# cvlab-kaist/SOLA

Hardware: AMD Instinct MI355X
Metric: track-selection forward+loss samples/sec at (T=32,N=64,d=256) (higher is better)
Workload: dtype f32 via split-f16 (hi+lo f16 operand pairs, 3 f16 MFMAs per product, f32 accumulate); 1 GPU; SOLA track selection forward+BCE+alignment loss+selection, T=32 N=64 d=256 L=16, mevis/default model (32.98M params, random init), 256 samples/step/GPU, conv weights re-standardised every step; batch_per_gpu=256, tracks=64, frames=32, text_len=16

## Files before the change

### include/sola_hip.h

```cpp
#ifndef SOLA_HIP_H
#define SOLA_HIP_H

#include <stddef.h>
#include <stdint.h>

#ifdef __cplusplus
extern "C" {
#endif

typedef enum SolaStatus {
    SOLA_OK = 0,
    SOLA_ERR_ARG = -1,
    SOLA_ERR_HIP = -2,
    SOLA_ERR_WEIGHT = -3,
    SOLA_ERR_WORKSPACE = -4,
    SOLA_ERR_STATE = -5
} SolaStatus;

typedef struct SolaConfig {
    int32_t object_token_dim;
    int32_t lang_token_dim;
    int32_t n_layers;
    int32_t max_temporal_length;
    int32_t n_negative;
    int32_t n_groups;
    int32_t n_groups_module;
    int32_t num_heads;
} SolaConfig;

typedef struct SolaCtx SolaCtx;

const char* sola_last_error(void);
const char* sola_version(void);

int sola_ctx_create(const SolaConfig* cfg, int device, SolaCtx** out);
int sola_ctx_destroy(SolaCtx* ctx);

int sola_num_weights(const SolaCtx* ctx);
int sola_weight_info(const SolaCtx* ctx, int index, const char** name, int64_t* numel);

int sola_set_weight(SolaCtx* ctx, const char* name, const void* dev_ptr, int64_t numel);

int sola_weights_changed(SolaCtx* ctx);
int sola_set_ws_policy(SolaCtx* ctx, int recompute_every_forward);

int sola_set_precision(SolaCtx* ctx, int precision);
int sola_set_split_guard(SolaCtx* ctx, int enable);

int sola_set_x16_arena(SolaCtx* ctx, void* dev_ptr, size_t bytes);
int sola_x16_arena_info(const SolaCtx* ctx, size_t* need_bytes, size_t* capacity_bytes, size_t* used_bytes);
int sola_split_fallback_count(const SolaCtx* ctx, int64_t* count, int32_t* last_guard);
int sola_cast_sp16(const float* dev_in, int ld_in, float* dev_out, int ld_out, int64_t rows, int K, float scale, void* stream);
int sola_cast_sp16_auto(const float* dev_in, int ld_in, float* dev_out, int ld_out, int64_t rows, int K, float* dev_scal, void* stream);
int sola_gemm_nt_split(const float* dev_a_sp, int lda, const float* dev_w_sp, const float* dev_bias, const float* dev_r,
                       int ldr, int r_is_split, float* dev_c, int ldc, int c_is_split, int M, int N, int K, float out_scale,
                       void* stream);
int sola_gemm_nt_split_scaled(const float* dev_a_sp, int lda, const float* dev_w_sp, const float* dev_bias, const float* dev_r,
                              int ldr, int r_is_split, float* dev_c, int ldc, int c_is_split, int M, int N, int K,
                              float out_scale, const float* dev_out_scale, void* stream);

int sola_cast_f16(const float* dev_in, int ld_in, void* dev_out, int ld_out, int64_t rows, int K, float scale, float* dev_scal, void* stream);
int sola_gemm_nt_f16(const void* dev_a_h, int lda, const void* dev_w_h, const float* dev_bias, const void* dev_r_h, int ldr,
                     void* dev_c, int ldc, int c_is_f16, int M, int N, int K, float out_scale, void* stream);
int sola_attention_f16(const void* dev_q, int ldq, const void* dev_k, int ldk, const void* dev_v, int ldv, void* dev_o, int ldo,
                       int G, int H, int head_dim, int Sq, int Sk, int inner, int64_t q_outer, int64_t q_inner, int64_t q_row_stride,
                       int64_t k_outer, int64_t k_inner, int64_t k_row_stride, float scale, void* stream);

int sola_gemm_nt_bf16(const void* dev_a, int lda, const void* dev_w, const float* dev_bias, const void* dev_r, int ldr, int r_is_bf16,
                      void* dev_c, int ldc, int c_is_bf16, int M, int N, int K, void* stream);
int sola_attention_bf16(const void* dev_q, int ldq, const void* dev_k, int ldk, const void* dev_v, int ldv, float* dev_o, void* dev_o_bf16, int ldo,
// ... 228 lines not shown
```

### sola_amd/_lib.py

```python
from __future__ import annotations

import contextlib
import ctypes as C
import os

_HERE = os.path.dirname(os.path.abspath(__file__))
LIB_PATH = os.environ.get("SOLA_HIP_LIB") or os.path.join(_HERE, "lib", "libsola_hip.so")


class SolaLibraryError(RuntimeError):
    pass


class SolaError(RuntimeError):
    """A libsola_hip call returned a negative status."""


class SolaConfig(C.Structure):
    _fields_ = [
        ("object_token_dim", C.c_int32),
        ("lang_token_dim", C.c_int32),
        ("n_layers", C.c_int32),
        ("max_temporal_length", C.c_int32),
        ("n_negative", C.c_int32),
# ... 8 lines not shown
        ("n_videos", C.c_int32),
        ("video_tracks", C.POINTER(C.c_int32)),
        ("video_frames", C.POINTER(C.c_int32)),
        ("n_samples", C.c_int32),
        ("sample_video", C.POINTER(C.c_int32)),
        ("sample_text_len", C.POINTER(C.c_int32)),
    ]


_vp, _i, _i64, _f, _sz = C.c_void_p, C.c_int, C.c_int64, C.c_float, C.c_size_t

SIGNATURES = {
    "sola_last_error": (C.c_char_p, []),
    "sola_version": (C.c_char_p, []),
    "sola_ctx_create": (_i, [C.POINTER(SolaConfig), _i, C.POINTER(_vp)]),
    "sola_ctx_destroy": (_i, [_vp]),
    "sola_num_weights": (_i, [_vp]),
    "sola_weight_info": (_i, [_vp, _i, C.POINTER(C.c_char_p), C.POINTER(_i64)]),
    "sola_set_weight": (_i, [_vp, C.c_char_p, _vp, _i64]),
    "sola_weights_changed": (_i, [_vp]),
    "sola_set_ws_policy": (_i, [_vp, _i]),
    "sola_set_precision": (_i, [_vp, _i]),
    "sola_set_split_guard": (_i, [_vp, _i]),
    "sola_split_fallback_count": (_i, [_vp, C.POINTER(_i64), C.POINTER(C.c_int32)]),
    "sola_cast_sp16": (_i, [_vp, _i, _vp, _i, _i64, _i, _f, _vp]),
    "sola_gemm_nt_split": (_i, [_vp, _i, _vp, _vp, _vp, _i, _i, _vp, _i, _i, _i, _i, _i, _f, _vp]),
    "sola_cast_sp16_auto": (_i, [_vp, _i, _vp, _i, _i64, _i, _vp, _vp]),
    "sola_gemm_nt_split_scaled": (_i, [_vp, _i, _vp, _vp, _vp, _i, _i, _vp, _i, _i, _i, _i, _i, _f, _vp, _vp]),
    "sola_cast_f16": (_i, [_vp, _i, _vp, _i, _i64, _i, _f, _vp, _vp]),
    "sola_gemm_nt_f16": (_i, [_vp, _i, _vp, _vp, _vp, _i, _vp, _i, _i, _i, _i, _i, _f, _vp]),
    "sola_gemm_nn": (_i, [_vp, _i, _vp, _vp, _vp, _i, _vp, _i, _vp, _i, _i, _i, _i, _vp]),
    "sola_gemm_nt_bf16": (_i, [_vp, _i, _vp, _vp, _vp, _i, _i, _vp, _i, _i, _i, _i, _i, _vp]),
    "sola_attention_bf16": (_i, [_vp, _i, _vp, _i, _vp, _i, _vp, _vp, _i, _i, _i, _i, _i, _i, _i, _i64, _i64, _i64, _i64, _i64, _i64, _f, _vp, _vp]),
    "sola_attention_backward_bf16": (_i, [_vp, _i, _vp, _i, _vp, _i, _vp, _i, _vp, _i, _i, _vp, _vp, _vp, _vp, _i, _i, _i, _vp, _vp, _i, _i, _i, _i, _i, _i,
                                          _i64, _i64, _i64, _i64, _i64, _i64, _f, _i64, _vp, _sz, _vp]),
    "sola_attention_f16": (_i, [_vp, _i, _vp, _i, _vp, _i, _vp, _i, _i, _i, _i, _i, _i, _i, _i64, _i64, _i64, _i64, _i64, _i64, _f, _vp]),
    "sola_workspace_bytes": (_sz, [_vp, _i, _i, _i, _i]),
    "sola_forward": (_i, [_vp, _vp, _vp, _i, _i, _i, _i, _vp, _vp, _vp, _sz, _vp]),
    "sola_ragged_workspace_bytes": (_sz, [_vp, C.POINTER(SolaRaggedBatch)]),
    "sola_forward_ragged": (_i, [_vp, _vp, _vp, C.POINTER(SolaRaggedBatch), _vp, _vp, _vp, _sz, _vp]),
    "sola_loss_ragged": (_i, [_vp, _vp, _vp, _vp, _vp, _i64, _i, _vp, _i, _i64, _i, _i, _f, _f, _f, _vp, _vp, _vp, _sz, _vp]),
    "sola_train_ragged_workspace_bytes": (_sz, [_vp, C.POINTER(SolaRaggedBatch)]),
    "sola_backward_ragged_workspace_bytes": (_sz, [_vp, C.POINTER(SolaRaggedBatch)]),
    "sola_forward_train_ragged": (_i, [_vp, _vp, _vp, C.POINTER(SolaRaggedBatch), _vp, _vp, _vp, _sz, _vp]),
    "sola_backward_ragged": (_i, [_vp, _vp, _vp, _vp, _vp, _sz, _vp]),
    "sola_loss_backward_ragged": (_i, [_vp, _vp, _vp, _vp, _vp, _i64, _i, _vp, _i, _i64, _i, _i, _f, _f, _f, _vp, _vp, _vp, _vp, _vp, _sz, _vp]),
# ... 179 lines not shown
```

### sola_amd/csrc/api.hip

```cpp
#include <math.h>
#include <stdarg.h>
#include <string.h>

#include <algorithm>
#include <exception>
#include <mutex>

#include "ragged.h"
#include "tune.h"

static thread_local char g_err[1024] = "";
void sola_set_error(const char* fmt, ...) {
    va_list ap;
    va_start(ap, fmt);
    vsnprintf(g_err, sizeof(g_err), fmt, ap);
    va_end(ap);
}
extern "C" const char* sola_last_error(void) { return g_err; }
extern "C" const char* sola_version(void) { return "sola_hip 0.6 (gfx950; f32, range-guarded split-f16 and f16-operand MFMA forward and backward, ragged batches, mask IoU + masklet rows)"; }

namespace {
struct ProfRec {
    int cat;
    hipEvent_t e0, e1;
// ... 577 lines not shown
                                const float* neg, int64_t neg_batch_stride, int n_samples, const int32_t* dev_track_offsets,
                                int max_tracks, int64_t total_tracks, int D, int n_neg, float pw, float temperature, float aw,
                                float* loss3, int32_t* neg_argmax, void* scratch, size_t scratch_bytes, void* stream_) {
    SOLA_ARG(score_map && score_tokens && labels && pos && neg && loss3 && scratch && dev_track_offsets, "loss_ragged: null argument");
    SOLA_ARG(n_samples > 0 && max_tracks > 0 && total_tracks > 0 && D > 0 && n_neg > 0, "loss_ragged: bad sizes");
    const size_t need = (size_t)total_tracks * 3 * sizeof(float);
    if (scratch_bytes < need) {
        sola_set_error("loss_ragged: scratch %zu bytes < required %zu", scratch_bytes, need);
        return SOLA_ERR_WORKSPACE;
    }
    LossDesc d{};
    d.score_map = score_map; d.score_tokens = score_tokens; d.labels = labels; d.pos = pos;
    d.neg = neg; d.neg_batch_stride = neg_batch_stride;
    d.B = n_samples; d.N = max_tracks; d.D = D; d.n_neg = n_neg;
    d.pos_w = pw; d.temp_scale = expf(temperature); d.align_w = aw;
    d.terms = static_cast<float*>(scratch); d.loss3 = loss3; d.neg_argmax = neg_argmax;
    d.trk_off = dev_track_offsets;
    return launch_loss(d, as_stream(stream_));
}

extern "C" int sola_set_split_guard(SolaCtx* c, int enable) {
    SOLA_ARG(c, "set_split_guard: null ctx");
    c->split_guard = enable != 0;
    return SOLA_OK;
}

extern "C" int sola_set_x16_arena(SolaCtx* c, void* dev_ptr, size_t bytes) {
    SOLA_ARG(c, "set_x16_arena: null ctx");
    SOLA_ARG((reinterpret_cast<uintptr_t>(dev_ptr) & 255) == 0, "set_x16_arena: the arena must be 256-byte aligned");
    c->x16.clear();
    c->x16_arena = static_cast<char*>(dev_ptr);
    c->x16_cap = dev_ptr ? bytes : 0;
    c->x16_used = 0;
    if (!dev_ptr) c->x16_need = 0;
    return SOLA_OK;
}

extern "C" int sola_x16_arena_info(const SolaCtx* c, size_t* need_bytes, size_t* capacity_bytes, size_t* used_bytes) {
    SOLA_ARG(c, "x16_arena_info: null ctx");
    if (need_bytes) *need_bytes = c->x16_need;
    if (capacity_bytes) *capacity_bytes = c->x16_cap;
    if (used_bytes) *used_bytes = c->x16_used;
    return SOLA_OK;
}

extern "C" int sola_split_fallback_count(const SolaCtx* c, int64_t* count, int32_t* last_guard) {
// ... 556 lines not shown
```

### sola_amd/csrc/backward.hip

```cpp
#include <math.h>
#include <stdlib.h>

#include <algorithm>
#include <initializer_list>
#include <string>
#include <vector>

#include "ragged.h"

extern int g_train_split_min_rows;
int g_bwd_dual_cast = 1;
int g_bwd_fused_bf16_cast = 1;

int g_train_dw_f16 = 1;
int g_bwd_side_rows = 0;
int g_bwd_group_rows = 2048;

namespace {

struct Arena {
    char* base;
    size_t total = 0;
    std::unordered_map<std::string, size_t> off, bytes;
    size_t add(const std::string& name, size_t floats) {
// ... 164 lines not shown
    const int max_rows_smp = rt ? rt->maxRowsSample : N * Tp;
    const float scale = 1.0f / sqrtf((float)DH);
    float* tn = ar.get("tn");
    const size_t tn_bytes = ar.total - ar.off.at("tn");
    float* wt = ar.get("wt");
    float* const splitk_ws = ar.off.count("splitk") ? ar.get("splitk") : nullptr;
    const size_t splitk_bytes = splitk_ws ? (size_t)8192 * 4096 * sizeof(float) : 0;
    const bool split = c->precision >= 1 && ar.off.count("dy_sp") != 0;
    const bool pure = c->precision >= 2;
    const int bf = c->precision == 3 ? 1 : 0;
    const int lowp_arith = pure ? 2 : 1;
    const bool dw16 = !pure && g_train_dw_f16 != 0;
    auto cast_scaled = [&](const float* in, int ld, float* out, long long rows, int K, float* scal) -> int {
        return pure ? launch_cast_f16_scaled(in, ld, out, K, rows, K, scal, s, bf) : launch_cast_sp16_scaled(in, ld, out, K, rows, K, scal, s);
    };
    auto cast_auto = [&](const float* in, int ld, float* out, long long rows, int K, float* scal) -> int {
        return pure ? launch_cast_f16(in, ld, out, K, rows, K, 0.f, scal, s, 13, nullptr, bf) : launch_cast_sp16_auto(in, ld, out, K, rows, K, scal, s);
    };
    auto cast_fixed = [&](const float* in, int ld, float* out, long long rows, int K, float scale) -> int {
        return pure ? launch_cast_f16(in, ld, out, K, rows, K, scale, nullptr, s, 13, nullptr, bf) : launch_cast_sp16(in, ld, out, K, rows, K, scale, s);
    };

    const bool lane_on = !split && g_bwd_side_rows > 0 && M <= g_bwd_side_rows;
    if (lane_on && !c->side_stream) {
        SOLA_HIP(hipStreamCreateWithFlags(&c->side_stream, hipStreamNonBlocking));
        SOLA_HIP(hipEventCreateWithFlags(&c->ev_fork, hipEventDisableTiming));
        for (hipEvent_t& e : c->ev_side) SOLA_HIP(hipEventCreateWithFlags(&e, hipEventDisableTiming));
    }
    hipStream_t s2 = lane_on ? c->side_stream : s;
    const bool group = !split && !lane_on && ar.off.count("dwkeep") != 0;
    float* keep_ptr = group ? ar.get("dwkeep") : nullptr;
    auto keep = [&](size_t floats) { float* q = keep_ptr; keep_ptr += (floats + 63) & ~(size_t)63; return q; };
    GemmTnGroupDesc gq{};
    auto flush_group = [&]() -> int {
        if (gq.nprob == 0) return SOLA_OK;
        SOLA_TRY(launch_gemm_tn_group(gq, s));
        gq.nprob = 0;
        return SOLA_OK;
    };
    const float* nn_w[3] = {nullptr, nullptr, nullptr};
    int nn_rows = 0;
    bool side_pending[4] = {false, false, false, false};
    auto dw_begin = [&]() -> int {
        if (!lane_on) return SOLA_OK;
        SOLA_HIP(hipEventRecord(c->ev_fork, s));
        SOLA_HIP(hipStreamWaitEvent(s2, c->ev_fork, 0));
        return SOLA_OK;
    };
    auto dw_end = [&](int slot) -> int {
        if (!lane_on) return SOLA_OK;
        SOLA_HIP(hipEventRecord(c->ev_side[slot], s2));
// ... 621 lines not shown
```

### sola_amd/csrc/ctx.h

```cpp
#pragma once
#include <string>
#include <unordered_map>
#include <vector>

#include "kernels.h"

struct ConvGeom {
    int cin, cout, k, stride, pad;
};
struct Weight {
    std::string name;
    int64_t numel;
    const float* ptr;
    float* grad;
};
struct Buf {
    size_t off;
    int64_t rows, cols;
};
struct Plan {
    int B = 0, N = 0, T = 0, L = 0, W = 0, Tp = 0, M = 0;
    int Tl[6] = {0};
    bool train = false;
    bool rag = false;
// ... 58 lines not shown
    void* x16_alloc(size_t bytes) {
        bytes = (bytes + 255) & ~(size_t)255;
        x16_need += bytes;
        if (x16_used + bytes > x16_cap) return nullptr;
        void* r = x16_arena + x16_used;
        x16_used += bytes;
        return r;
    }
    const void* x16_find(const float* src, int cols, int fmt) const {
        for (const X16Entry& e : x16)
            if (e.src == src && e.cols == cols && e.fmt == fmt) return e.p16;
        return nullptr;
    }
    float* scal_buf = nullptr;
    int* guard = nullptr;
    int* guard_host = nullptr;
    bool split_guard = true;
    long long split_fallbacks = 0;
    bool weight_range_bad = false;
    SolaRagStage* rag_stage = nullptr;
    std::vector<hipEvent_t> bucket_ev;
    hipStream_t side_stream = nullptr;
    hipEvent_t ev_fork = nullptr, ev_side[4] = {nullptr, nullptr, nullptr, nullptr};
    bool bucket_recorded = false;
    int n_buckets() const { return cfg.n_layers + 1; }
    float* scal_pair(int i) const { return scal_buf + 2 * i; }
    float* scal_extra(int i) const { return scal_buf + 2 * (2 + (size_t)cfg.n_layers * 12) + 2 + i; }
    const float* lin_inv_scale(int layer, int attn, int proj) const { return scal_buf + 2 * (2 + (layer * 3 + attn) * 4 + proj) + 1; }
    struct StepBinding {
        std::vector<int> widx;
        std::vector<int32_t> group;
        std::vector<long long> numel;
        int n_groups = 0;
        size_t sq_scratch = 0;
    } step;
    void* adam_tab = nullptr;
    int adam_n = 0, adam_cap = 0, adam_blocks = 0;
    bool adam_has_steps = false;
    int* adam_ticket = nullptr;
    double adam_bytes = 0.0;
    float p_drop_encoder = 0.f, p_drop_attention = 0.f;
    unsigned long long drop_seed = 0;
    DropoutCfg enc_drop(int conv_idx) const { return make_dropout(p_drop_encoder, drop_seed, 1u + (unsigned)conv_idx); }
    DropoutCfg attn_drop(int layer, int a) const { return make_dropout(p_drop_attention, drop_seed, 100u + 3u * (unsigned)layer + (unsigned)a); }
};

static const int kConvIdx[6] = {0, 4, 8, 12, 16, 20};
static const int kNormIdx[5] = {1, 5, 9, 13, 17};
static const char* const kAttnShort[3] = {"obj", "mot", "o2l"};
static const char* const kAttnLong[3] = {"obj_attn", "motion_attn", "object2lang_attn"};
constexpr float kLinScale = 64.f;
int sola_refresh_lin16(SolaCtx* c, hipStream_t s);
int sola_refresh_conv_weights(SolaCtx* c, int fmt, bool force, hipStream_t s);
int sola_check_forward_args(const SolaCtx* c, const char* who, size_t need, const void* workspace, size_t ws_bytes);

inline const float* ctx_weight(const SolaCtx* c, const std::string& name) {
    auto it = c->index.find(name);
    return it == c->index.end() ? nullptr : c->weights[it->second].ptr;
}
inline float* ctx_grad(const SolaCtx* c, const std::string& name) {
    auto it = c->index.find(name);
    return it == c->index.end() ? nullptr : c->weights[it->second].grad;
}

inline std::string abuf(bool train, int layer, const char* attn, const char* what) {
    if (!train) return what;
    return "l" + std::to_string(layer) + "_" + attn + "_" + what;
}

struct RagShape;
Plan make_plan(const SolaCtx* c, int B, int N, int T, int L, bool train);
Plan make_plan_ragged(const SolaCtx* c, const RagShape& r, bool train);
int sola_forward_train_impl(SolaCtx* c, const float* obj, const float* lang, int B, int N, int T, int L, float* score_map,
                            float* score_tokens, void* workspace, size_t ws_bytes, hipStream_t s, const RagShape* rs = nullptr);
int sola_forward_infer_impl(SolaCtx* c, const float* obj, const float* lang, int B, int N, int T, int L, float* score_map,
                            float* score_tokens, void* workspace, size_t ws_bytes, hipStream_t s);
// ... 5 lines not shown
```

### sola_amd/csrc/forward.hip

```cpp
#include <math.h>
#include <string.h>

#include <algorithm>

#include "ragged.h"

int g_train_gn_cast = 1;
extern int g_train_dw_f16;
int g_train_attn_cast = 1;
int g_train_bf16_store = 3;
int g_train_gn_stats = 1;
int g_train_x16_keep = 1;
int g_train_split_min_rows = 1024;

namespace {
struct PlanSizes {
    int64_t rows0;
    int64_t rows[6];
    int64_t M, BW;
    int64_t S;
    int64_t gn_slots;
    size_t tables;
};
void plan_fill(Plan& p, const SolaCtx* c, const PlanSizes& z, bool train) {
// ... 43 lines not shown
        p.add("l" + std::to_string(l) + "_o2l", z.M, D);
    }
}
}

Plan make_plan(const SolaCtx* c, int B, int N, int T, int L, bool train) {
    Plan p;
    p.B = B; p.N = N; p.T = T; p.L = L; p.train = train;
    p.W = L + c->cfg.n_negative;
    int t = T;
    for (int i = 0; i < 6; ++i) {
        t = (t + 2 * c->conv[i].pad - c->conv[i].k) / c->conv[i].stride + 1;
        p.Tl[i] = t;
    }
    p.Tp = p.Tl[5];
    p.M = B * N * p.Tp;
    const int64_t R = (int64_t)B * N;
    PlanSizes z{};
    z.rows0 = R * T;
    for (int i = 0; i < 6; ++i) z.rows[i] = R * p.Tl[i];
    z.M = p.M; z.BW = (int64_t)B * p.W; z.S = B;
    z.gn_slots = std::max<int64_t>(R * T, (int64_t)p.M) / 4 + 1024;
    plan_fill(p, c, z, train);
    return p;
}

Plan make_plan_ragged(const SolaCtx* c, const RagShape& r, bool train) {
    Plan p;
    p.rag = true;
    p.B = r.S; p.N = r.maxN; p.T = r.maxT[0]; p.L = r.maxW - c->cfg.n_negative; p.train = train;
    p.W = r.maxW;
    for (int i = 0; i < 6; ++i) p.Tl[i] = r.maxT[i + 1];
    p.Tp = r.maxT[6];
    p.M = (int)r.Ms;
    PlanSizes z{};
    z.rows0 = r.rows[0];
    for (int i = 0; i < 6; ++i) z.rows[i] = r.rows[i + 1];
    z.M = r.Ms; z.BW = r.LW; z.S = r.S;
    z.gn_slots = (int64_t)(rag_gn_slots_bytes(r) / 4 + 64);
    z.tables = rag_tables_bytes(r, train);
    plan_fill(p, c, z, train);
    return p;
}

int sola_forward_train_impl(SolaCtx* c, const float* obj, const float* lang, int B, int N, int T, int L, float* score_map,
                            float* score_tokens, void* workspace, size_t ws_bytes, hipStream_t s, const RagShape* rs) {
// ... 351 lines not shown
```

### sola_amd/csrc/forward_infer.hip

```cpp
#include <math.h>

#include <algorithm>

#include "ctx.h"

int sola_refresh_lin16(SolaCtx* c, hipStream_t s) {
    if (!c->lin16_dirty) return SOLA_OK;
    SOLA_ARG(c->lin16_buf && c->scal_buf, "split-f16 weights requested before sola_set_precision(ctx, 1)");
    static const char* pn[4] = {"q_proj", "k_proj", "v_proj", "out_proj"};
    const int D = c->cfg.lang_token_dim;
    std::vector<const float*> in;
    std::vector<float*> out;
    for (int l = 0; l < c->cfg.n_layers; ++l)
        for (int a = 0; a < 3; ++a)
            for (int j = 0; j < 4; ++j) {
                const std::string nm = "object_lang_align_layers." + std::to_string(l) + "." + kAttnLong[a] + "." + pn[j] + ".weight";
                const float* w = ctx_weight(c, nm);
                if (!w) {
                    sola_set_error("forward: weight '%s' has not been set", nm.c_str());
                    return SOLA_ERR_WEIGHT;
                }
                in.push_back(w);
                out.push_back(c->lin16_buf + ((size_t)(l * 3 + a) * 4 + j) * D * D);
            }
// ... 46 lines not shown
    c->ws16_fmt = fmt;
    return SOLA_OK;
}

int sola_check_forward_args(const SolaCtx* c, const char* who, size_t need, const void* workspace, size_t ws_bytes) {
    for (const Weight& w : c->weights)
        if (!w.ptr) {
            sola_set_error("%s: weight '%s' has not been set", who, w.name.c_str());
            return SOLA_ERR_WEIGHT;
        }
    if (ws_bytes < need) {
        sola_set_error("%s: workspace %zu bytes < required %zu", who, ws_bytes, need);
        return SOLA_ERR_WORKSPACE;
    }
    SOLA_ARG((reinterpret_cast<uintptr_t>(workspace) & 255) == 0, "%s: workspace must be 256-byte aligned", who);
    return SOLA_OK;
}

int g_attn_split_min_keys = 96;

int g_lang_shared_neg = 1;

int launch_attention_f16(const AttnDesc& d, hipStream_t s);

int sola_forward_infer_impl(SolaCtx* c, const float* obj, const float* lang, int B, int N, int T, int L, float* score_map,
                            float* score_tokens, void* workspace, size_t ws_bytes, hipStream_t s) {
    SOLA_ARG(c && obj && lang && score_map && score_tokens && workspace, "forward: null argument");
    SOLA_ARG(B > 0 && N > 0 && T > 0 && L >= 1, "forward: bad sizes B=%d N=%d T=%d L=%d", B, N, T, L);
    const bool sp = c->precision == 1;
    const bool h16 = c->precision == 2;
    if (sp)
        SOLA_ARG(c->cfg.object_token_dim % 8 == 0 && (c->cfg.lang_token_dim / c->cfg.n_groups_module) % 8 == 0 &&
                     (2 * c->cfg.object_token_dim / c->cfg.n_groups) % 8 == 0 && (c->cfg.lang_token_dim / c->cfg.n_groups) % 8 == 0,
                 "split-f16 mode needs channel counts per GroupNorm group that are multiples of 8");
    if (h16)
        SOLA_ARG(c->cfg.object_token_dim % 64 == 0 && c->cfg.lang_token_dim % 64 == 0,
                 "16-bit storage mode needs object_token_dim and lang_token_dim to be multiples of 64");
    Plan p = make_plan(c, B, N, T, L, false);
    SOLA_TRY(sola_check_forward_args(c, "forward", p.total, workspace, ws_bytes));
    char* base = static_cast<char*>(workspace);
    auto buf = [&](const std::string& name) { return reinterpret_cast<float*>(base + p.bufs.at(name).off); };
    float* const splitk_ws = (!h16 && p.bufs.count("splitk")) ? buf("splitk") : nullptr;
    const size_t splitk_bytes = splitk_ws ? (size_t)p.bufs.at("splitk").rows * p.bufs.at("splitk").cols * sizeof(float) : 0;
    auto W = [&](const std::string& name) { return ctx_weight(c, name); };
    const int D = c->cfg.lang_token_dim, H = c->cfg.num_heads, DH = D / H, d_in = c->cfg.object_token_dim;
    const int Tp = p.Tp, M = p.M, Wn = p.W;
    const int R = B * N;
    int* const guard = (sp || h16) ? c->guard : nullptr;
    auto ws_w = [&](int i) -> const float* {
        if (h16) return reinterpret_cast<const float*>(reinterpret_cast<const _Float16*>(c->ws16_buf) + c->ws_off[i]);
        return sp ? c->ws16_buf + c->ws_off[i] : c->ws_buf + c->ws_off[i];
    };
    auto lin_w = [&](const std::string& an, const char* proj_name, int layer, int attn, int proj) -> const float* {
        const size_t idx = (size_t)(layer * 3 + attn) * 4 + proj;
        if (sp) return c->lin16_buf + idx * D * D;
        if (h16) return reinterpret_cast<const float*>(reinterpret_cast<const _Float16*>(c->lin16_buf) + idx * D * D);
        return W(an + "." + proj_name + ".weight");
    };
    auto lin_inv = [&](int layer, int attn, int proj) -> const float* { return (sp || h16) ? c->lin_inv_scale(layer, attn, proj) : nullptr; };

    SOLA_TRY(sola_refresh_conv_weights(c, sp ? 1 : (h16 ? 2 : 0), false, s));
    if (sp || h16) {
        SOLA_TRY(sola_refresh_lin16(c, s));
        SOLA_HIP(hipMemsetAsync(c->guard, 0, sizeof(int), s));
    } else {
        c->x16.clear();
        c->x16_used = 0;
        c->x16_need = 0;
    }

    const float* x = obj;
    if (sp) SOLA_TRY(launch_cast_sp16_auto(obj, d_in, buf("obj_sp"), d_in, (long long)R * T, d_in, c->scal_pair(0), s));
    if (h16) SOLA_TRY(launch_cast_f16(obj, d_in, buf("obj_sp"), d_in, (long long)R * T, d_in, 256.f, c->scal_pair(0), s, 6, c->scal_extra(0)));
    if (sp || h16) x = buf("obj_sp");
    const bool conv5_16 = h16 || (sp && c->conv[5].cout % 8 == 0);
    int t_in = T;
    for (int i = 0; i < 6; ++i) {
        const ConvGeom& g = c->conv[i];
        const std::string cp = "short_motion_encoder." + std::to_string(kConvIdx[i]);
        const bool to16 = i == 5 && conv5_16;
        GemmDesc gd{};
        gd.nprob = 1;
        gd.p[0] = GemmProblem{x, ws_w(i), W(cp + ".bias"), nullptr, to16 ? buf("conv5_sp") : buf("conv" + std::to_string(i))};
        gd.M = R * p.Tl[i]; gd.N = g.cout; gd.K = g.k * g.cin;
        gd.lda = g.cin; gd.ldr = 0; gd.ldc = g.cout;
        gd.conv = g.k > 1 ? 1 : 0;
        gd.T_in = t_in; gd.T_out = p.Tl[i]; gd.stride = g.stride; gd.pad = g.pad; gd.Cin = g.cin;
        if (sp) {
            gd.arith = 1; gd.out_scale = 1.f; gd.c_sp16 = to16 ? 1 : 0; gd.guard = guard;
            if (i == 0) gd.out_scale_dev = c->scal_pair(0) + 1;
        }
        if (h16) {
            gd.arith = 2; gd.out_scale = 1.f; gd.c_f16 = 1; gd.guard = guard;
            if (i == 0) gd.bias_scale_dev = c->scal_extra(0);
        }
        gd.splitk_ws = splitk_ws; gd.splitk_bytes = splitk_bytes;
        bool fused_norm = false;
// ... 10 lines not shown
            }
        }
        SOLA_TRY(launch_gemm(gd, s));
        if (i < 5 && !fused_norm) {
            const std::string np = "short_motion_encoder." + std::to_string(kNormIdx[i]);
            GroupNormDesc nd{};
            nd.slice_ws = buf("gn_slots"); nd.slice_ws_bytes = (size_t)p.bufs.at("gn_slots").rows * p.bufs.at("gn_slots").cols * sizeof(float);
            nd.x = buf("conv" + std::to_string(i)); nd.y = buf("act" + std::to_string(i));
            nd.gamma = W(np + ".weight"); nd.beta = W(np + ".bias");
            nd.n_inst = R; nd.inner = 1; nd.outer_stride = p.Tl[i]; nd.inner_stride = 0; nd.tok_stride = 1;
            nd.ntok = p.Tl[i]; nd.C = g.cout; nd.groups = c->cfg.n_groups; nd.eps = 1e-5f; nd.slope = 0.01f; nd.leaky = 1;
            nd.out_sp16 = sp ? 1 : 0; nd.guard = guard;
            if (h16) {
                nd.in_f16 = 1; nd.out_f16 = 1;
                if (i == 0) nd.in_scale_dev = c->scal_pair(0) + 1;
            }
            SOLA_TRY(launch_group_norm(nd, s));
        }
        if (i < 5) x = buf("act" + std::to_string(i));
        t_in = p.Tl[i];
    }
    if (sp && !conv5_16) SOLA_TRY(launch_cast_sp16(buf("conv5"), D, buf("conv5_sp"), D, M, D, 1.f, s));

    SOLA_TRY(launch_pos_encoding(W("positional_encoding_gaussian_matrix"), D, Tp, c->cfg.max_temporal_length, buf("pe"), s));
    bool shared_neg = false;
    if (sp && g_lang_shared_neg && c->cfg.n_negative > 0 && Wn <= g_attn_split_min_keys && (long long)B * L + c->cfg.n_negative >= 1024) {
        AttnDesc probe{};
        probe.G = B; probe.H = H; probe.DH = DH; probe.Sq = N * Tp; probe.Sk = Wn; probe.inner = 1; probe.k_private = L;
        shared_neg = attention_shared_keys_supported(probe);
    }
    const long long lang_rows = shared_neg ? (long long)B * L + c->cfg.n_negative : (long long)B * Wn;
    if (shared_neg) SOLA_TRY(launch_lang_concat_shared(lang, W("negative_token.weight"), buf("lang"), buf("lbar"), B, L, c->cfg.n_negative, D, s));
    else SOLA_TRY(launch_lang_concat(lang, W("negative_token.weight"), buf("lang"), buf("lbar"), B, L, c->cfg.n_negative, D, s));
    if (sp) SOLA_TRY(launch_cast_sp16_auto(buf("lang"), D, buf("lang_sp"), D, lang_rows, D, c->scal_pair(1), s));
    if (h16) SOLA_TRY(launch_cast_f16(buf("lang"), D, buf("lang_sp"), D, lang_rows, D, 1.f, c->scal_pair(1), s, 6));
    const float* const lang_in = (sp || h16) ? buf("lang_sp") : buf("lang");

    const float scale = 1.0f / sqrtf((float)DH);
    auto linear3 = [&](const float* a0, const float* a1, const float* a2, int layer, int attn, int nprob, int rows, float* o0,
                       float* o1, float* o2, int first_proj, int out_sp16, const float* a_inv_scale = nullptr) -> int {
        static const char* pn[3] = {"q_proj", "k_proj", "v_proj"};
        const std::string an = "object_lang_align_layers." + std::to_string(layer) + "." + kAttnLong[attn];
        const float* as[3] = {a0, a1, a2};
        float* os[3] = {o0, o1, o2};
        GemmDesc gd{};
        gd.nprob = nprob;
        for (int j = 0; j < nprob; ++j)
            gd.p[j] = GemmProblem{as[j], lin_w(an, pn[first_proj + j], layer, attn, first_proj + j), W(an + "." + pn[first_proj + j] + ".bias"),
                                  nullptr, os[j], lin_inv(layer, attn, first_proj + j)};
        gd.M = rows; gd.N = D; gd.K = D; gd.lda = D; gd.ldr = 0; gd.ldc = D;
        if (sp) { gd.arith = 1; gd.out_scale = 1.f; gd.out_scale_dev = a_inv_scale; gd.c_sp16 = out_sp16; gd.guard = guard; }
        if (h16) { gd.arith = 2; gd.out_scale = 1.f; gd.out_scale_dev = a_inv_scale; gd.c_f16 = 1; gd.guard = guard; }
        gd.splitk_ws = splitk_ws; gd.splitk_bytes = splitk_bytes;
        return launch_gemm(gd, s);
    };
    auto out_proj = [&](int layer, int attn, const float* resid, int resid_sp16) -> int {
        const std::string an = "object_lang_align_layers." + std::to_string(layer) + "." + kAttnLong[attn];
        GemmDesc gd{};
        gd.nprob = 1;
        gd.p[0] = GemmProblem{buf("attn"), lin_w(an, "out_proj", layer, attn, 3), W(an + ".out_proj.bias"), resid, buf("res"), lin_inv(layer, attn, 3)};
        gd.M = M; gd.N = D; gd.K = D; gd.lda = D; gd.ldr = D; gd.ldc = D;
        if (sp) { gd.arith = 1; gd.out_scale = 1.f; gd.r_sp16 = resid_sp16; }
        if (h16) { gd.arith = 2; gd.out_scale = 1.f; gd.r_f16 = 1; gd.c_f16 = 1; gd.guard = guard; }
        gd.splitk_ws = splitk_ws; gd.splitk_bytes = splitk_bytes;
        return launch_gemm(gd, s);
    };
    auto gn = [&](const std::string& lp, int idx, float* y, float* y2, int out16, int n_inst, int inner, long long outer,
                  long long inner_stride, long long tok_stride, int ntok) -> int {
        GroupNormDesc nd{};
        nd.slice_ws = buf("gn_slots"); nd.slice_ws_bytes = (size_t)p.bufs.at("gn_slots").rows * p.bufs.at("gn_slots").cols * sizeof(float);
        nd.x = buf("res"); nd.y = y; nd.y2 = y2; nd.pe = y2 ? buf("pe") : nullptr;
        nd.gamma = W(lp + "norm." + std::to_string(idx) + ".weight");
        nd.beta = W(lp + "norm." + std::to_string(idx) + ".bias");
        nd.n_inst = n_inst; nd.inner = inner; nd.outer_stride = outer; nd.inner_stride = inner_stride;
        nd.tok_stride = tok_stride; nd.ntok = ntok; nd.C = D; nd.groups = c->cfg.n_groups_module;
        nd.eps = 1e-5f; nd.slope = 0.f; nd.leaky = 0; nd.guard = guard;
        if (sp) nd.out_sp16 = out16;
        if (h16) { nd.in_f16 = 1; nd.out_f16 = out16; }
        return launch_group_norm(nd, s);
    };
    auto attention = [&](const float* q, const float* k, const float* v, int G, int Sq, int Sk, int inner, long long qo,
                         long long qi, long long qr, long long ko, long long ki, long long kr, int in_sp16, int k_private = 0,
                         long long k_shared_row = 0) -> int {
        AttnDesc ad{q, k, v, buf("attn"), D, D, D, D, G, H, DH, Sq, Sk, inner, qo, qi, qr, ko, ki, kr, scale, nullptr};
        ad.k_private = k_private;
        ad.k_shared_row = k_shared_row;
        ad.o_sp16 = sp ? 1 : 0;
        ad.in_sp16 = in_sp16;
        ad.guard = guard;
        ad.split_math = sp ? 1 : 0;
        return h16 ? launch_attention_f16(ad, s) : launch_attention(ad, s);
    };
    const int obj_sp = (sp && N > g_attn_split_min_keys && N > 16 && DH % 16 == 0) ? 1 : 0;
    const int mot_sp = (sp && Tp > g_attn_split_min_keys && Tp > 16 && DH % 16 == 0) ? 1 : 0;
    const int o2l_sp = (sp && Wn > g_attn_split_min_keys && DH % 16 == 0) ? 1 : 0;

    const float* xin = (sp || h16) ? buf("conv5_sp") : buf("conv5");
    const float* xres = conv5_16 ? buf("conv5_sp") : buf("conv5");
    int xres_sp = conv5_16 ? 1 : 0;
    for (int l = 0; l < c->cfg.n_layers; ++l) {
        const std::string lp = "object_lang_align_layers." + std::to_string(l) + ".";
        const std::string ls = "l" + std::to_string(l);
        const bool last = l + 1 == c->cfg.n_layers;
        float *q = buf("q"), *k = buf("k"), *v = buf("v");
        float* x_obj = buf(ls + "_obj");
        float* x_pe = buf(ls + "_xpe");
        float* x_mot = buf(ls + "_motion");
        float* x_o2l = buf(ls + "_o2l");
        SOLA_TRY(linear3(xin, xin, xin, l, 0, 3, M, q, k, v, 0, obj_sp));
        SOLA_TRY(attention(q, k, v, B * Tp, N, N, Tp, (long long)N * Tp, 1, Tp, (long long)N * Tp, 1, Tp, obj_sp));
        SOLA_TRY(out_proj(l, 0, xres, xres_sp));
        SOLA_TRY(gn(lp, 0, x_obj, x_pe, 1, B * Tp, Tp, (long long)N * Tp, 1, Tp, N));
        SOLA_TRY(linear3(x_pe, x_pe, x_obj, l, 1, 3, M, q, k, v, 0, mot_sp));
        SOLA_TRY(attention(q, k, v, B * N, Tp, Tp, 1, (long long)Tp, 0, 1, (long long)Tp, 0, 1, mot_sp));
        SOLA_TRY(out_proj(l, 1, x_obj, 1));
        SOLA_TRY(gn(lp, 1, x_mot, nullptr, 1, B * N, 1, Tp, 0, 1, Tp));
        SOLA_TRY(linear3(x_mot, nullptr, nullptr, l, 2, 1, M, q, nullptr, nullptr, 0, o2l_sp));
        SOLA_TRY(linear3(lang_in, lang_in, nullptr, l, 2, 2, (int)lang_rows, buf("lk"), buf("lv"), nullptr, 1, o2l_sp, c->scal_pair(1) + 1));
        if (shared_neg) SOLA_TRY(attention(q, buf("lk"), buf("lv"), B, N * Tp, Wn, 1, (long long)N * Tp, 0, 1, (long long)L, 0, 1, o2l_sp, L, (long long)B * L));
        else SOLA_TRY(attention(q, buf("lk"), buf("lv"), B, N * Tp, Wn, 1, (long long)N * Tp, 0, 1, (long long)Wn, 0, 1, o2l_sp));
        SOLA_TRY(out_proj(l, 2, x_mot, 1));
        SOLA_TRY(gn(lp, 2, x_o2l, nullptr, last ? 0 : 1, B, 1, (long long)N * Tp, 0, 1, N * Tp));
        xin = x_o2l;
        xres = x_o2l;
        xres_sp = 1;
    }

    HeadDesc hd{xin, buf("lbar"), score_map, score_tokens, B, N, Tp, D};
    SOLA_TRY(launch_score_head(hd, s));
    c->last = p;
    c->last_obj = nullptr;
    return SOLA_OK;
}
```

### sola_amd/module.py

```python
from __future__ import annotations

import ctypes as C

import os

import torch
import torch.nn as nn

from . import _lib
from ._lib import SolaConfig, SolaError, SolaRaggedBatch, check, current_stream, lib, ptr, require_cuda

NUM_HEADS = 8


class _AttentionParams(nn.Module):

    def __init__(self, embed_dim, num_heads, dropout_p=0.1):
        super().__init__()
        self.embed_dim, self.num_heads, self.dropout_p = embed_dim, num_heads, dropout_p
        self.q_proj = nn.Linear(embed_dim, embed_dim)
        self.k_proj = nn.Linear(embed_dim, embed_dim)
        self.v_proj = nn.Linear(embed_dim, embed_dim)
        self.out_proj = nn.Linear(embed_dim, embed_dim)

# ... 62 lines not shown
        mods = []
        for cin, cout, k, s, pad in geo:
            mods += [nn.Conv1d(cin, cout, kernel_size=k, stride=s, padding=pad),
                     nn.GroupNorm(self.n_groups, cout), nn.LeakyReLU(), nn.Dropout(p=p)]
        mods.append(nn.Conv1d(D, D, kernel_size=1, stride=1, padding=0))
        self.short_motion_encoder = nn.Sequential(*mods)
        self.object_lang_align_layers = nn.ModuleList([ObjectLanguageAlignmentLayer(configs) for _ in range(self.n_layers)])
        self.register_buffer("positional_encoding_gaussian_matrix", torch.randn((1, D // 2)).float())
        self.negative_token = nn.Embedding(self.n_negative, D)
        self._ctx = None
        self._ctx_device = None
        self._bound = {}
        self._weights_touched = False
        self._workspace = None
        self._last_shape = None
        self.ws_policy = "auto"
        self.attention_dropout_p = 0.1
        env = os.environ.get("SOLA_PRECISION")
        self._precision = env or "f16x3"
        self.train_precision = os.environ.get("SOLA_TRAIN_PRECISION") or env or "f32"
        self._ctx_precision = None
        self.split_guard = True
        self._ctx_guard = None
        self._train_ws = None
        self._bwd_ws = None
        self._train_inputs = None
        self._train_shape = None
        self._train_generation = 0
        self._grad_arena = None
        self._grad_ctx = None
        self._grad_bound = None
        self._grads_in_arena = False

    def _config_struct(self):
        return SolaConfig(self.object_token_dim, self.lang_token_dim, self.n_layers, self.max_temporal_length,
                          self.n_negative, self.n_groups, self.n_groups_module, NUM_HEADS)

    def _ensure_ctx(self, device):
        if self._ctx is not None and self._ctx_device == device:
            return
        self._release_ctx()
        handle = C.c_void_p()
        cfg = self._config_struct()
        check(lib().sola_ctx_create(C.byref(cfg), device.index if device.index is not None else torch.cuda.current_device(),
                                    C.byref(handle)), "sola_ctx_create")
        self._ctx, self._ctx_device, self._bound = handle, device, {}
        self._ctx_precision = None
        self._ctx_guard = None

    def _release_ctx(self):
        if getattr(self, "_ctx", None) is not None:
            try:
                lib().sola_ctx_destroy(self._ctx)
            finally:
                self._ctx = None

    def __del__(self):
        try:
            self._release_ctx()
        except Exception:
            pass

    def _params(self):
        return [(key, owner._parameters[leaf]) for key, owner, leaf, is_buf in self._state_entries() if not is_buf]

    def _param_list(self):
        return [p for _, p in self._params()]

    def _state_entries(self):
        se = self.__dict__.get("_state_cache")
        if se is None:
# ... 29 lines not shown
            rec = (t.data_ptr(), t._version)
            old = self._bound.get(key)
            if old is None or old[0] != rec[0]:
                check(lib().sola_set_weight(self._ctx, key.encode(), ptr(t), t.numel()), f"sola_set_weight({key})")
                self._adam_sig = None
                changed = True
            elif old[1] != rec[1]:
                changed = True
            self._bound[key] = rec
        if changed:
            check(lib().sola_weights_changed(self._ctx), "sola_weights_changed")
        every = self.training if self.ws_policy == "auto" else self.ws_policy == "always"
        check(lib().sola_set_ws_policy(self._ctx, 1 if every else 0), "sola_set_ws_policy")
        prec = self.train_precision if train else self._precision
        if prec not in ("f32", "f16x3", "f16", "bf16"):
            raise SolaError(f"precision must be 'f32', 'f16x3', 'f16' or 'bf16', got {prec!r}")
        want = {"f32": 0, "f16x3": 1, "f16": 2, "bf16": 3 if train else 1}[prec]
        if self._ctx_precision != want:
            check(lib().sola_set_precision(self._ctx, want), "sola_set_precision")
            self._ctx_precision = want
        if self._ctx_guard != bool(self.split_guard):
            check(lib().sola_set_split_guard(self._ctx, 1 if self.split_guard else 0), "sola_set_split_guard")
            self._ctx_guard = bool(self.split_guard)

    def split_fallbacks(self):
        if self._ctx is None:
            return 0, 0
        n, g = C.c_int64(), C.c_int32()
        check(lib().sola_split_fallback_count(self._ctx, C.byref(n), C.byref(g)), "sola_split_fallback_count")
        return int(n.value), int(g.value)

    def _get_workspace(self, nbytes, device):
        if self._workspace is None or self._workspace.numel() < nbytes or self._workspace.device != device:
            self._workspace = torch.empty(int(nbytes), dtype=torch.uint8, device=device)
        return self._workspace

    def _check_inputs(self, object_tokens, lang_tokens):
        if object_tokens.dim() != 4 or lang_tokens.dim() != 3:
            raise SolaError("object_tokens must be [B,N,T,d] and lang_tokens [B,L,D]")
        B, N, T, d = object_tokens.shape
        Bl, L, D = lang_tokens.shape
        if d != self.object_token_dim or D != self.lang_token_dim or Bl != B:
            raise SolaError(f"shape mismatch: object_tokens {tuple(object_tokens.shape)}, lang_tokens {tuple(lang_tokens.shape)}")
        if min(B, N, T, L) < 1:
            raise SolaError(f"empty input: object_tokens {tuple(object_tokens.shape)}, lang_tokens {tuple(lang_tokens.shape)}")

# ... 503 lines not shown
```

Baseline: 18520 samples/s.

## Overlap conv weight refresh and language K/V projections on a side stream in inference

```diff
diff --git a/include/sola_hip.h b/include/sola_hip.h
--- a/include/sola_hip.h
+++ b/include/sola_hip.h
@@ -46,6 +46,8 @@
 
 int sola_set_precision(SolaCtx* ctx, int precision);
 int sola_set_split_guard(SolaCtx* ctx, int enable);
+
+int sola_set_infer_side_stream(SolaCtx* ctx, int enable);
 
 int sola_set_x16_arena(SolaCtx* ctx, void* dev_ptr, size_t bytes);
 int sola_x16_arena_info(const SolaCtx* ctx, size_t* need_bytes, size_t* capacity_bytes, size_t* used_bytes);
diff --git a/sola_amd/_lib.py b/sola_amd/_lib.py
--- a/sola_amd/_lib.py
+++ b/sola_amd/_lib.py
@@ -54,6 +54,7 @@
     "sola_set_ws_policy": (_i, [_vp, _i]),
     "sola_set_precision": (_i, [_vp, _i]),
     "sola_set_split_guard": (_i, [_vp, _i]),
+    "sola_set_infer_side_stream": (_i, [_vp, _i]),
     "sola_split_fallback_count": (_i, [_vp, C.POINTER(_i64), C.POINTER(C.c_int32)]),
     "sola_cast_sp16": (_i, [_vp, _i, _vp, _i, _i64, _i, _f, _vp]),
     "sola_gemm_nt_split": (_i, [_vp, _i, _vp, _vp, _vp, _i, _i, _vp, _i, _i, _i, _i, _i, _f, _vp]),
diff --git a/sola_amd/csrc/api.hip b/sola_amd/csrc/api.hip
--- a/sola_amd/csrc/api.hip
+++ b/sola_amd/csrc/api.hip
@@ -623,6 +623,12 @@
 extern "C" int sola_set_split_guard(SolaCtx* c, int enable) {
     SOLA_ARG(c, "set_split_guard: null ctx");
     c->split_guard = enable != 0;
+    return SOLA_OK;
+}
+
+extern "C" int sola_set_infer_side_stream(SolaCtx* c, int enable) {
+    SOLA_ARG(c, "set_infer_side_stream: null ctx");
+    c->infer_side = enable != 0;
     return SOLA_OK;
 }
 
diff --git a/sola_amd/csrc/backward.hip b/sola_amd/csrc/backward.hip
--- a/sola_amd/csrc/backward.hip
+++ b/sola_amd/csrc/backward.hip
@@ -210,11 +210,7 @@
     };
 
     const bool lane_on = !split && g_bwd_side_rows > 0 && M <= g_bwd_side_rows;
-    if (lane_on && !c->side_stream) {
-        SOLA_HIP(hipStreamCreateWithFlags(&c->side_stream, hipStreamNonBlocking));
-        SOLA_HIP(hipEventCreateWithFlags(&c->ev_fork, hipEventDisableTiming));
-        for (hipEvent_t& e : c->ev_side) SOLA_HIP(hipEventCreateWithFlags(&e, hipEventDisableTiming));
-    }
+    if (lane_on) SOLA_TRY(sola_side_lane_init(c));
     hipStream_t s2 = lane_on ? c->side_stream : s;
     const bool group = !split && !lane_on && ar.off.count("dwkeep") != 0;
     float* keep_ptr = group ? ar.get("dwkeep") : nullptr;
diff --git a/sola_amd/csrc/ctx.h b/sola_amd/csrc/ctx.h
--- a/sola_amd/csrc/ctx.h
+++ b/sola_amd/csrc/ctx.h
@@ -104,6 +104,7 @@
     std::vector<hipEvent_t> bucket_ev;
     hipStream_t side_stream = nullptr;
     hipEvent_t ev_fork = nullptr, ev_side[4] = {nullptr, nullptr, nullptr, nullptr};
+    bool infer_side = true;
     bool bucket_recorded = false;
     int n_buckets() const { return cfg.n_layers + 1; }
     float* scal_pair(int i) const { return scal_buf + 2 * i; }
@@ -134,6 +135,7 @@
 constexpr float kLinScale = 64.f;
 int sola_refresh_lin16(SolaCtx* c, hipStream_t s);
 int sola_refresh_conv_weights(SolaCtx* c, int fmt, bool force, hipStream_t s);
+int sola_side_lane_init(SolaCtx* c);
 int sola_check_forward_args(const SolaCtx* c, const char* who, size_t need, const void* workspace, size_t ws_bytes);
 
 inline const float* ctx_weight(const SolaCtx* c, const std::string& name) {
diff --git a/sola_amd/csrc/forward.hip b/sola_amd/csrc/forward.hip
--- a/sola_amd/csrc/forward.hip
+++ b/sola_amd/csrc/forward.hip
@@ -89,6 +89,13 @@
     z.M = p.M; z.BW = (int64_t)B * p.W; z.S = B;
     z.gn_slots = std::max<int64_t>(R * T, (int64_t)p.M) / 4 + 1024;
     plan_fill(p, c, z, train);
+    if (!train) {
+        for (int l = 1; l < c->cfg.n_layers; ++l) {
+            p.add("l" + std::to_string(l) + "_lk", z.BW, c->cfg.lang_token_dim);
+            p.add("l" + std::to_string(l) + "_lv", z.BW, c->cfg.lang_token_dim);
+        }
+        if (p.bufs.count("splitk")) p.add("splitk_side", p.bufs.at("splitk").rows, p.bufs.at("splitk").cols);
+    }
     return p;
 }
 
diff --git a/sola_amd/csrc/forward_infer.hip b/sola_amd/csrc/forward_infer.hip
--- a/sola_amd/csrc/forward_infer.hip
+++ b/sola_amd/csrc/forward_infer.hip
@@ -92,6 +92,52 @@
 int g_lang_shared_neg = 1;
 
 int launch_attention_f16(const AttnDesc& d, hipStream_t s);
+
+int sola_side_lane_init(SolaCtx* c) {
+    if (c->side_stream) return SOLA_OK;
+    SOLA_HIP(hipStreamCreateWithFlags(&c->side_stream, hipStreamNonBlocking));
+    SOLA_HIP(hipEventCreateWithFlags(&c->ev_fork, hipEventDisableTiming));
+    for (hipEvent_t& e : c->ev_side) SOLA_HIP(hipEventCreateWithFlags(&e, hipEventDisableTiming));
+    return SOLA_OK;
+}
+
+namespace {
+struct SideLane {
+    SolaCtx* c;
+    hipStream_t s;
+    bool open = false;
+    SideLane(SolaCtx* c_, hipStream_t s_) : c(c_), s(s_) {}
+    SideLane(const SideLane&) = delete;
+    SideLane& operator=(const SideLane&) = delete;
+    int fork() {
+        SOLA_TRY(sola_side_lane_init(c));
+        SOLA_HIP(hipEventRecord(c->ev_fork, s));
+        SOLA_HIP(hipStreamWaitEvent(c->side_stream, c->ev_fork, 0));
+        open = true;
+        return SOLA_OK;
+    }
+    int mark(int slot) {
+        SOLA_HIP(hipEventRecord(c->ev_side[slot], c->side_stream));
+        return SOLA_OK;
+    }
+    int wait(int slot) {
+        SOLA_HIP(hipStreamWaitEvent(s, c->ev_side[slot], 0));
+        return SOLA_OK;
+    }
+    int join() {
+        open = false;
+        SOLA_TRY(mark(1));
+        return wait(1);
+    }
+    ~SideLane() {
+        if (open) (void)join();
+    }
+};
+bool stream_is_capturing(hipStream_t s) {
+    hipStreamCaptureStatus st = hipStreamCaptureStatusNone;
+    return hipStreamIsCapturing(s, &st) != hipSuccess || st != hipStreamCaptureStatusNone;
+}
+}
 
 int sola_forward_infer_impl(SolaCtx* c, const float* obj, const float* lang, int B, int N, int T, int L, float* score_map,
                             float* score_tokens, void* workspace, size_t ws_bytes, hipStream_t s) {
@@ -129,7 +175,9 @@
     };
     auto lin_inv = [&](int layer, int attn, int proj) -> const float* { return (sp || h16) ? c->lin_inv_scale(layer, attn, proj) : nullptr; };
 
-    SOLA_TRY(sola_refresh_conv_weights(c, sp ? 1 : (h16 ? 2 : 0), false, s));
+    const bool side = c->infer_side && !stream_is_capturing(s);
+    SideLane lane(c, s);
+    if (!side) SOLA_TRY(sola_refresh_conv_weights(c, sp ? 1 : (h16 ? 2 : 0), false, s));
     if (sp || h16) {
         SOLA_TRY(sola_refresh_lin16(c, s));
         SOLA_HIP(hipMemsetAsync(c->guard, 0, sizeof(int), s));
@@ -139,10 +187,68 @@
         c->x16_need = 0;
     }
 
+    bool shared_neg = false;
+    if (sp && g_lang_shared_neg && c->cfg.n_negative > 0 && Wn <= g_attn_split_min_keys && (long long)B * L + c->cfg.n_negative >= 1024) {
+        AttnDesc probe{};
+        probe.G = B; probe.H = H; probe.DH = DH; probe.Sq = N * Tp; probe.Sk = Wn; probe.inner = 1; probe.k_private = L;
+        shared_neg = attention_shared_keys_supported(probe);
+    }
+    const long long lang_rows = shared_neg ? (long long)B * L + c->cfg.n_negative : (long long)B * Wn;
+    const float* const lang_in = (sp || h16) ? buf("lang_sp") : buf("lang");
+    const int o2l_sp = (sp && Wn > g_attn_split_min_keys && DH % 16 == 0) ? 1 : 0;
+    auto text_front = [&](hipStream_t st) -> int {
+        SOLA_TRY(launch_pos_encoding(W("positional_encoding_gaussian_matrix"), D, Tp, c->cfg.max_temporal_length, buf("pe"), st));
+        if (shared_neg) SOLA_TRY(launch_lang_concat_shared(lang, W("negative_token.weight"), buf("lang"), buf("lbar"), B, L, c->cfg.n_negative, D, st));
+        else SOLA_TRY(launch_lang_concat(lang, W("negative_token.weight"), buf("lang"), buf("lbar"), B, L, c->cfg.n_negative, D, st));
+        if (sp) SOLA_TRY(launch_cast_sp16_auto(buf("lang"), D, buf("lang_sp"), D, lang_rows, D, c->scal_pair(1), st));
+        if (h16) SOLA_TRY(launch_cast_f16(buf("lang"), D, buf("lang_sp"), D, lang_rows, D, 1.f, c->scal_pair(1), st, 6));
+        return SOLA_OK;
+    };
+    auto linear3_on = [&](hipStream_t st, float* sk_ws, const float* a0, const float* a1, const float* a2, int layer, int attn, int nprob, int rows,
+                          float* o0, float* o1, float* o2, int first_proj, int out_sp16, const float* a_inv_scale) -> int {
+        static const char* pn[3] = {"q_proj", "k_proj", "v_proj"};
+        const std::string an = "object_lang_align_layers." + std::to_string(layer) + "." + kAttnLong[attn];
+        const float* as[3] = {a0, a1, a2};
+        float* os[3] = {o0, o1, o2};
+        GemmDesc gd{};
+        gd.nprob = nprob;
+        for (int j = 0; j < nprob; ++j)
+            gd.p[j] = GemmProblem{as[j], lin_w(an, pn[first_proj + j], layer, attn, first_proj + j), W(an + "." + pn[first_proj + j] + ".bias"),
+                                  nullptr, os[j], lin_inv(layer, attn, first_proj + j)};
+        gd.M = rows; gd.N = D; gd.K = D; gd.lda = D; gd.ldr = 0; gd.ldc = D;
+        if (sp) { gd.arith = 1; gd.out_scale = 1.f; gd.out_scale_dev = a_inv_scale; gd.c_sp16 = out_sp16; gd.guard = guard; }
+        if (h16) { gd.arith = 2; gd.out_scale = 1.f; gd.out_scale_dev = a_inv_scale; gd.c_f16 = 1; gd.guard = guard; }
+        gd.splitk_ws = sk_ws; gd.splitk_bytes = splitk_bytes;
+        return launch_gemm(gd, st);
+    };
+    auto linear3 = [&](const float* a0, const float* a1, const float* a2, int layer, int attn, int nprob, int rows, float* o0, float* o1,
+                       float* o2, int first_proj, int out_sp16) -> int {
+        return linear3_on(s, splitk_ws, a0, a1, a2, layer, attn, nprob, rows, o0, o1, o2, first_proj, out_sp16, nullptr);
+    };
+    auto lang_k = [&](int l) { return l == 0 ? buf("lk") : buf("l" + std::to_string(l) + "_lk"); };
+    auto lang_v = [&](int l) { return l == 0 ? buf("lv") : buf("l" + std::to_string(l) + "_lv"); };
+    auto lang_kv_proj = [&](int l, hipStream_t st, float* sk_ws) -> int {
+        return linear3_on(st, sk_ws, lang_in, lang_in, nullptr, l, 2, 2, (int)lang_rows, lang_k(l), lang_v(l), nullptr, 1, o2l_sp, c->scal_pair(1) + 1);
+    };
+    auto side_front = [&]() -> int {
+        hipStream_t s2 = c->side_stream;
+        SOLA_TRY(sola_refresh_conv_weights(c, sp ? 1 : (h16 ? 2 : 0), false, s2));
+        SOLA_TRY(lane.mark(0));
+        SOLA_TRY(text_front(s2));
+        float* const sk2 = splitk_ws ? buf("splitk_side") : nullptr;
+        for (int l = 0; l < c->cfg.n_layers; ++l) SOLA_TRY(lang_kv_proj(l, s2, sk2));
+        return SOLA_OK;
+    };
+    if (side) SOLA_TRY(lane.fork());
+
     const float* x = obj;
     if (sp) SOLA_TRY(launch_cast_sp16_auto(obj, d_in, buf("obj_sp"), d_in, (long long)R * T, d_in, c->scal_pair(0), s));
     if (h16) SOLA_TRY(launch_cast_f16(obj, d_in, buf("obj_sp"), d_in, (long long)R * T, d_in, 256.f, c->scal_pair(0), s, 6, c->scal_extra(0)));
     if (sp || h16) x = buf("obj_sp");
+    if (side) {
+        SOLA_TRY(side_front());
+        SOLA_TRY(lane.wait(0));
+    }
     const bool conv5_16 = h16 || (sp && c->conv[5].cout % 8 == 0);
     int t_in = T;
     for (int i = 0; i < 6; ++i) {
@@ -199,38 +305,7 @@
     }
     if (sp && !conv5_16) SOLA_TRY(launch_cast_sp16(buf("conv5"), D, buf("conv5_sp"), D, M, D, 1.f, s));
 
-    SOLA_TRY(launch_pos_encoding(W("positional_encoding_gaussian_matrix"), D, Tp, c->cfg.max_temporal_length, buf("pe"), s));
-    bool shared_neg = false;
-    if (sp && g_lang_shared_neg && c->cfg.n_negative > 0 && Wn <= g_attn_split_min_keys && (long long)B * L + c->cfg.n_negative >= 1024) {
-        AttnDesc probe{};
-        probe.G = B; probe.H = H; probe.DH = DH; probe.Sq = N * Tp; probe.Sk = Wn; probe.inner = 1; probe.k_private = L;
-        shared_neg = attention_shared_keys_supported(probe);
-    }
-    const long long lang_rows = shared_neg ? (long long)B * L + c->cfg.n_negative : (long long)B * Wn;
-    if (shared_neg) SOLA_TRY(launch_lang_concat_shared(lang, W("negative_token.weight"), buf("lang"), buf("lbar"), B, L, c->cfg.n_negative, D, s));
-    else SOLA_TRY(launch_lang_concat(lang, W("negative_token.weight"), buf("lang"), buf("lbar"), B, L, c->cfg.n_negative, D, s));
-    if (sp) SOLA_TRY(launch_cast_sp16_auto(buf("lang"), D, buf("lang_sp"), D, lang_rows, D, c->scal_pair(1), s));
-    if (h16) SOLA_TRY(launch_cast_f16(buf("lang"), D, buf("lang_sp"), D, lang_rows, D, 1.f, c->scal_pair(1), s, 6));
-    const float* const lang_in = (sp || h16) ? buf("lang_sp") : buf("lang");
-
     const float scale = 1.0f / sqrtf((float)DH);
-    auto linear3 = [&](const float* a0, const float* a1, const float* a2, int layer, int attn, int nprob, int rows, float* o0,
-                       float* o1, float* o2, int first_proj, int out_sp16, const float* a_inv_scale = nullptr) -> int {
-        static const char* pn[3] = {"q_proj", "k_proj", "v_proj"};
-        const std::string an = "object_lang_align_layers." + std::to_string(layer) + "." + kAttnLong[attn];
-        const float* as[3] = {a0, a1, a2};
-        float* os[3] = {o0, o1, o2};
-        GemmDesc gd{};
-        gd.nprob = nprob;
-        for (int j = 0; j < nprob; ++j)
-            gd.p[j] = GemmProblem{as[j], lin_w(an, pn[first_proj + j], layer, attn, first_proj + j), W(an + "." + pn[first_proj + j] + ".bias"),
-                                  nullptr, os[j], lin_inv(layer, attn, first_proj + j)};
-        gd.M = rows; gd.N = D; gd.K = D; gd.lda = D; gd.ldr = 0; gd.ldc = D;
-        if (sp) { gd.arith = 1; gd.out_scale = 1.f; gd.out_scale_dev = a_inv_scale; gd.c_sp16 = out_sp16; gd.guard = guard; }
-        if (h16) { gd.arith = 2; gd.out_scale = 1.f; gd.out_scale_dev = a_inv_scale; gd.c_f16 = 1; gd.guard = guard; }
-        gd.splitk_ws = splitk_ws; gd.splitk_bytes = splitk_bytes;
-        return launch_gemm(gd, s);
-    };
     auto out_proj = [&](int layer, int attn, const float* resid, int resid_sp16) -> int {
         const std::string an = "object_lang_align_layers." + std::to_string(layer) + "." + kAttnLong[attn];
         GemmDesc gd{};
@@ -270,8 +345,9 @@
     };
     const int obj_sp = (sp && N > g_attn_split_min_keys && N > 16 && DH % 16 == 0) ? 1 : 0;
     const int mot_sp = (sp && Tp > g_attn_split_min_keys && Tp > 16 && DH % 16 == 0) ? 1 : 0;
-    const int o2l_sp = (sp && Wn > g_attn_split_min_keys && DH % 16 == 0) ? 1 : 0;
-
+
+    if (side) SOLA_TRY(lane.join());
+    else SOLA_TRY(text_front(s));
     const float* xin = (sp || h16) ? buf("conv5_sp") : buf("conv5");
     const float* xres = conv5_16 ? buf("conv5_sp") : buf("conv5");
     int xres_sp = conv5_16 ? 1 : 0;
@@ -293,9 +369,9 @@
         SOLA_TRY(out_proj(l, 1, x_obj, 1));
         SOLA_TRY(gn(lp, 1, x_mot, nullptr, 1, B * N, 1, Tp, 0, 1, Tp));
         SOLA_TRY(linear3(x_mot, nullptr, nullptr, l, 2, 1, M, q, nullptr, nullptr, 0, o2l_sp));
-        SOLA_TRY(linear3(lang_in, lang_in, nullptr, l, 2, 2, (int)lang_rows, buf("lk"), buf("lv"), nullptr, 1, o2l_sp, c->scal_pair(1) + 1));
-        if (shared_neg) SOLA_TRY(attention(q, buf("lk"), buf("lv"), B, N * Tp, Wn, 1, (long long)N * Tp, 0, 1, (long long)L, 0, 1, o2l_sp, L, (long long)B * L));
-        else SOLA_TRY(attention(q, buf("lk"), buf("lv"), B, N * Tp, Wn, 1, (long long)N * Tp, 0, 1, (long long)Wn, 0, 1, o2l_sp));
+        if (!side) SOLA_TRY(lang_kv_proj(l, s, splitk_ws));
+        if (shared_neg) SOLA_TRY(attention(q, lang_k(l), lang_v(l), B, N * Tp, Wn, 1, (long long)N * Tp, 0, 1, (long long)L, 0, 1, o2l_sp, L, (long long)B * L));
+        else SOLA_TRY(attention(q, lang_k(l), lang_v(l), B, N * Tp, Wn, 1, (long long)N * Tp, 0, 1, (long long)Wn, 0, 1, o2l_sp));
         SOLA_TRY(out_proj(l, 2, x_mot, 1));
         SOLA_TRY(gn(lp, 2, x_o2l, nullptr, last ? 0 : 1, B, 1, (long long)N * Tp, 0, 1, N * Tp));
         xin = x_o2l;
diff --git a/sola_amd/module.py b/sola_amd/module.py
--- a/sola_amd/module.py
+++ b/sola_amd/module.py
@@ -108,6 +108,8 @@
         self._ctx_precision = None
         self.split_guard = True
         self._ctx_guard = None
+        self.side_stream = os.environ.get("SOLA_INFER_SIDE_STREAM", "1") != "0"
+        self._ctx_side = None
         self._train_ws = None
         self._bwd_ws = None
         self._train_inputs = None
@@ -133,6 +135,7 @@
         self._ctx, self._ctx_device, self._bound = handle, device, {}
         self._ctx_precision = None
         self._ctx_guard = None
+        self._ctx_side = None
 
     def _release_ctx(self):
         if getattr(self, "_ctx", None) is not None:
@@ -208,6 +211,9 @@
         if self._ctx_guard != bool(self.split_guard):
             check(lib().sola_set_split_guard(self._ctx, 1 if self.split_guard else 0), "sola_set_split_guard")
             self._ctx_guard = bool(self.split_guard)
+        if self._ctx_side != bool(self.side_stream):
+            check(lib().sola_set_infer_side_stream(self._ctx, 1 if self.side_stream else 0), "sola_set_infer_side_stream")
+            self._ctx_side = bool(self.side_stream)
 
     def split_fallbacks(self):
         if self._ctx is None:
```

Result: no change. 18710 samples/s, median of 6 (+1.0%).
